# magenta/ddsp

Measured on NVIDIA H100. Metric: audio samples/sec (Harmonic+FilteredNoise decoder), higher is better.
Workload: dtype f32

## Files before the change

### ddsp_b200/csrc/noise_ring.cuh

```cuda
#pragma once
#include "noise_fused.cuh"

namespace ddsp {

namespace nr_ {
constexpr int NB = 65, FRAME = 64, S = 128, S0 = 128, Q = 32, SHIFT = 64;
constexpr int R = 16;
constexpr int UPT = FRAME / R;
constexpr int CONS_WARPS = 8, PROD_GROUPS = 3;
constexpr int GROUP_WARPS = 4, PROD_WARPS = GROUP_WARPS * PROD_GROUPS;
constexpr int NTG = CONS_WARPS / UPT;
static_assert((NTG & (NTG - 1)) == 0, "tile groups: a power of two");
constexpr int SLOTS = 7;
static_assert(SLOTS > NTG + 1, "the ring must leave slots to the producers");
constexpr int RING = 32 * SLOTS;
constexpr int THREADS = 32 * (CONS_WARPS + PROD_WARPS);
static_assert(THREADS <= 640, "noise_ring: the FIR needs 96 registers per thread");
constexpr int HPAD = 2, HS = 134, XS = 66, MS = 65;
constexpr int NQ = FRAME / 4;

constexpr int E_STEPS = 9, O_STEPS = 8;
constexpr int E_NT = 5, O_NT = 4;
constexpr int TAB_E = E_STEPS * E_NT * 32, TAB = TAB_E + O_STEPS * O_NT * 32;
__host__ __device__ constexpr int ir_kk(int s, int t) { return 16 * (s >> 2) + 4 * t + (s & 3); }

#ifdef DDSP_NR_TIMING
#define NR_TIMING_DECL unsigned tprev__ = (unsigned)clock()
__device__ unsigned g_nr_timing[kMaxSMs * 32 * 8];
#define NR_LAP(i)                                                                       \
  do {                                                                                  \
    const unsigned n__ = (unsigned)clock();                                             \
    if (lane == 0) atomicAdd(&g_nr_timing[(blockIdx.x * 32 + warp) * 8 + (i)], n__ - tprev__); \
    tprev__ = n__;                                                                      \
  } while (0)
#else
#define NR_TIMING_DECL
#define NR_LAP(i)
#endif

struct Smem {
  double ctab[TAB];
  float win[S];
  alignas(16) float raw[PROD_GROUPS][32 * NB + 8];
  alignas(16) float h[RING * HS];
  alignas(16) float x[RING * XS];
  alignas(8) unsigned long long full[SLOTS], empty[SLOTS], rawbar[PROD_GROUPS];
};

struct Params {
  const float* __restrict__ mags;
  const float* __restrict__ noise;
  float* audio;
  uint64_t seed, offset;
  int B, F, N, accumulate, raw, item_base;
  float bias;
};

struct Seg {
  int b, s0, len, nP, nC;
};

__device__ __forceinline__ bool next_seg(long long& g, long long g1, int F, Seg& sg) {
  if (g >= g1) return false;
  sg.b = (int)(g / F);
  sg.s0 = (int)(g - (long long)sg.b * F);
  sg.len = (int)min((long long)(F - sg.s0), g1 - g);
  sg.nP = (sg.len + 3 + 31) >> 5;
  sg.nC = (sg.len + 31) >> 5;
  g += sg.len;
  return true;
}

__device__ __forceinline__ void mbar_arrive_n(void* bar, int n) {
  asm volatile("mbarrier.arrive.shared::cta.b64 _, [%0], %1;" ::"r"(smem_u32(bar)),
               "r"(n)
               : "memory");
}

__device__ __forceinline__ float4 lds128v(const float* p) {
  float4 v;
  asm volatile("ld.shared.v4.f32 {%0, %1, %2, %3}, [%4];"
               : "=f"(v.x), "=f"(v.y), "=f"(v.z), "=f"(v.w)
               : "r"(smem_u32(p)));
  return v;
}
__device__ __forceinline__ float lds32v(const float* p) {
  float v;
  asm volatile("ld.shared.f32 %0, [%1];" : "=f"(v) : "r"(smem_u32(p)));
  return v;
}

__device__ __forceinline__ void dmma_16x8x4(double (&d)[4], double a0, double a1, double b) {
  asm("mma.sync.aligned.m16n8k4.row.col.f64.f64.f64.f64 {%0, %1, %2, %3}, {%4, %5}, {%6}, "
      "{%0, %1, %2, %3};"
      : "+d"(d[0]), "+d"(d[1]), "+d"(d[2]), "+d"(d[3])
      : "d"(a0), "d"(a1), "d"(b));
}

__device__ __forceinline__ void red_add_v4(float* addr, float a, float b, float c,
                                           float d) {
  asm volatile("red.global.add.v4.f32 [%0], {%1, %2, %3, %4};" ::"l"(addr), "f"(a),
               "f"(b), "f"(c), "f"(d)
               : "memory");
}

extern __shared__ __align__(16) unsigned char nr_smem[];
constexpr int X_OFF = (int)(offsetof(Smem, x) / 4), H_OFF = (int)(offsetof(Smem, h) / 4);
__device__ __forceinline__ float lds1(int off) {
  return reinterpret_cast<const float*>(nr_smem)[off];
}
__device__ __forceinline__ float2 lds2(int off) {
  return *reinterpret_cast<const float2*>(reinterpret_cast<const float*>(nr_smem) + off);
}

template <int D, int DLO, int DHI>
__device__ __forceinline__ void fir_diag(float (&y)[R], const float (&X)[R], float t) {
  if constexpr (D >= DLO && D <= DHI) {
#pragma unroll
    for (int k = (D < 0 ? -D : 0); k < (D > 0 ? R - D : R); ++k)
      y[k + D] = fmaf(X[k], t, y[k + D]);
  }
}
template <int J, int DLO, int DHI>
__device__ __forceinline__ void fir_pairs(float (&y)[R], const float (&X)[R], int ho) {
  if constexpr (2 * J + 1 >= DLO) {
    const float2 P = lds2(ho + 2 * J);
    fir_diag<2 * J + 1, DLO, DHI>(y, X, P.y);
    fir_diag<2 * J, DLO, DHI>(y, X, P.x);
    fir_pairs<J - 1, DLO, DHI>(y, X, ho);
  }
}
template <int DLO, int DHI>
__device__ __forceinline__ void fir_body(float (&y)[R], int xo, int ho) {
  float X[R];
#pragma unroll
  for (int k = 0; k < R; k += 2) {
    const float2 v = lds2(xo + k);
    X[k] = v.x;
    X[k + 1] = v.y;
  }
  fir_pairs<DHI / 2, DLO, DHI>(y, X, ho);
}

enum { OP_FULL = 0, OP_LOWER = 1, OP_UPPER = 2 };
constexpr int N_OPS = 2 * UPT + 1;

__device__ __forceinline__ void consume_unit(float (&y)[R], int u, const int (&xr)[4],
                                             const int (&hr)[4]) {
  const int N0 = R * u;
  const int xm1 = xr[0], hm1 = hr[0], x0 = xr[1], h0 = hr[1], xp1 = xr[2], hp1 = hr[2];
#pragma unroll 1
  for (int i = 0; i < N_OPS; ++i) {
    int kind = OP_FULL, xo, ho;
    if (i < UPT) {
      xo = x0 + R * i;
      ho = h0 + N0 + 62 - R * i;
    } else if (i < UPT + u) {
      const int j = i - UPT;
      xo = xm1 + R * j;
      ho = hm1 + N0 - 2 - R * j;
    } else if (i == UPT + u) {
      kind = OP_LOWER;
      xo = xm1 + N0;
      ho = hm1 - 2;
    } else if (i == UPT + u + 1) {
      kind = OP_UPPER;
      xo = xp1 + N0;
      ho = hp1 + 126;
    } else {
      const int j = i - UPT - 1;
      xo = xp1 + R * j;
      ho = hp1 + N0 + 126 - R * j;
    }
    switch (kind) {
      case OP_FULL: fir_body<-(R - 1), R - 1>(y, xo, ho); break;
      case OP_LOWER: fir_body<2, R - 1>(y, xo, ho); break;
      default: fir_body<-(R - 1), 1>(y, xo, ho); break;
    }
  }
  const int xe = u ? xp1 + N0 - 1 : xr[3] + 63, he = u ? hp1 + 127 : hr[3] + 127;
  y[0] = fmaf(lds1(xe), lds1(he), y[0]);
}
__global__ void __launch_bounds__(nr_::THREADS, 1)
noise_ring_kernel(Params p) {
  Smem& sm = *reinterpret_cast<Smem*>(nr_smem);
  const int tid = threadIdx.x, lane = tid & 31, warp = tid >> 5;

  for (int e = tid; e < TAB; e += THREADS) {
    const bool even = e < TAB_E;
    const int ee = even ? e : e - TAB_E, nts = even ? E_NT : O_NT;
    const int l = ee & 31, s = (ee >> 5) / nts, nt = (ee >> 5) - s * nts;
    const int kk = ir_kk(s, l & 3), k = even ? 2 * kk : 2 * kk + 1, n = 8 * nt + (l >> 2);
    double v = 0.0;
    if (k < NB && n <= Q) {
      const double ck = (k == 0 || k == NB - 1) ? 1.0 : 2.0;
      v = ck / S0 * cospi(2.0 * (double)((k * n) % S0) / S0);
    }
    sm.ctab[e] = v;
  }
  for (int j = tid; j < S; j += THREADS)
    sm.win[j] = 0.5f - 0.5f * cospif(2.0f * (float)j / (float)S0);
  for (int e = tid; e < RING * HS; e += THREADS) sm.h[e] = 0.f;
  for (int e = tid; e < RING * XS; e += THREADS) sm.x[e] = 0.f;
#ifdef DDSP_NR_TIMING
  for (int e = tid; e < 32 * 8; e += THREADS) g_nr_timing[blockIdx.x * 32 * 8 + e] = 0;
#endif
  if (tid == 0) {
    for (int i = 0; i < SLOTS; ++i) {
      mbar_init(&sm.full[i], GROUP_WARPS);
      mbar_init(&sm.empty[i], 2 * UPT);
    }
    for (int i = 0; i < PROD_GROUPS; ++i) mbar_init(&sm.rawbar[i], 1);
  }
  __syncthreads();

  const long long T = (long long)p.B * p.F;
  const long long g_lo = T * blockIdx.x / gridDim.x;
  const long long g_hi = T * (blockIdx.x + 1) / gridDim.x;

  if (warp < CONS_WARPS) {
    const int tg = warp / UPT, unit = warp % UPT;
    long long g = g_lo;
    Seg sg;
    int pbase = 0, ct = 0;
    bool dep_done = false;
    NR_TIMING_DECL;
    while (next_seg(g, g_hi, p.F, sg)) {
      for (int t = (tg - ct) & (NTG - 1); t < sg.nC; t += NTG) {
        NR_LAP(3);
        {
          const int P0 = pbase + t, P1 = pbase + min(t + 1, sg.nP - 1);
          mbar_wait(&sm.full[P0 % SLOTS], (P0 / SLOTS) & 1);
          mbar_wait(&sm.full[P1 % SLOTS], (P1 / SLOTS) & 1);
        }
        NR_LAP(0);
        const int q_rel = 32 * t + lane;
        const int rho = min(q_rel, sg.len - 1) + 2;
        const int rbase = pbase * 32;
        int xr[4], hr[4];
#pragma unroll
        for (int s = 0; s < 4; ++s) {
          const int row = (rbase + rho + 1 - s) % RING;
          xr[s] = X_OFF + row * XS;
          hr[s] = H_OFF + row * HS + HPAD;
        }
        float y[R];
#pragma unroll
        for (int c = 0; c < R; ++c) y[c] = 0.f;
        consume_unit(y, unit, xr, hr);
        __syncwarp();
        NR_LAP(1);
        if (lane == 0) {
#pragma unroll
          for (int d = 0; d < 2; ++d) {
            const int tau = t + d;
            if (tau < sg.nP) {
              const int readers = (tau >= 1 ? 1 : 0) + (tau < sg.nC ? 1 : 0);
              mbar_arrive_n(&sm.empty[(pbase + tau) % SLOTS], 2 / readers);
            }
          }
        }
        if (!dep_done) {
          asm volatile("griddepcontrol.wait;" ::: "memory");
          dep_done = true;
        }
        if (q_rel < sg.len) {
          constexpr int NOUT = R;
          const long long t0 = (long long)(sg.s0 + q_rel) * FRAME + NOUT * unit;
          float* o = p.audio + (size_t)sg.b * p.N + t0;
          if (t0 + NOUT <= p.N && (reinterpret_cast<uintptr_t>(o) & 15) == 0) {
#pragma unroll
            for (int w4 = 0; w4 < NOUT / 4; ++w4) {
              if (p.accumulate)
                red_add_v4(o + 4 * w4, y[4 * w4], y[4 * w4 + 1], y[4 * w4 + 2],
                           y[4 * w4 + 3]);
              else
                *reinterpret_cast<float4*>(o + 4 * w4) =
                    make_float4(y[4 * w4], y[4 * w4 + 1], y[4 * w4 + 2], y[4 * w4 + 3]);
            }
          } else {
#pragma unroll
            for (int w1 = 0; w1 < NOUT; ++w1) {
              if (t0 + w1 < p.N) {
                if (p.accumulate) o[w1] += y[w1]; else o[w1] = y[w1];
              }
            }
          }
        }
        NR_LAP(2);
      }
      ct += sg.nC;
      pbase += sg.nP;
    }
  } else {
    const int grp = (warp - CONS_WARPS) / GROUP_WARPS;
    const int iw = (warp - CONS_WARPS) % GROUP_WARPS;
    const int ptid = tid - (CONS_WARPS + GROUP_WARPS * grp) * 32;
    constexpr int PT = 32 * GROUP_WARPS;
    const int bar_id = 1 + grp;
    float* s_raw = sm.raw[grp];
    void* rawbar = &sm.rawbar[grp];
    const float* mags_end = p.mags + (size_t)p.B * p.F * NB;
    auto prefetch = [&](const Seg& s, int tau) -> int {
      const int jb = s.s0 - 2 + 32 * tau;
      const int r_lo = max(0, -jb), r_hi = min(32, p.F - jb);
      if (r_hi <= r_lo) {
        if (ptid == 0) mbar_arrive(rawbar);
        return 0;
      }
      const float* src = p.mags + ((size_t)s.b * p.F + jb + r_lo) * NB;
      const uintptr_t a = reinterpret_cast<uintptr_t>(src);
      const int off = (int)((a & 15) >> 2);
      const uint32_t bytes = (uint32_t)(((off + (r_hi - r_lo) * NB) * 4 + 15) & ~15);
      const uintptr_t a_al = a & ~(uintptr_t)15;
      if (a_al >= reinterpret_cast<uintptr_t>(p.mags) &&
          a_al + bytes <= reinterpret_cast<uintptr_t>(mags_end)) {
        if (ptid == 0) {
          mbar_expect_tx(rawbar, bytes);
          tma_bulk_g2s(s_raw, reinterpret_cast<const void*>(a_al), bytes, rawbar);
        }
        return off - r_lo * NB;
      }
      for (int e = ptid; e < (r_hi - r_lo) * NB; e += PT) cp_async4(s_raw + e, src + e);
      cp_async_wait_all();
      named_bar(bar_id, PT);
      if (ptid == 0) mbar_arrive(rawbar);
      return -r_lo * NB;
    };
    struct It {
      long long g;
      Seg sg;
      int tau, P;
      bool ok;
    };
    auto it_begin = [&]() {
      It it;
      it.g = g_lo; it.tau = 0; it.P = 0;
      it.ok = next_seg(it.g, g_hi, p.F, it.sg);
      return it;
    };
    auto it_next = [&](It& it) {
      ++it.P;
      if (++it.tau >= it.sg.nP) {
        it.tau = 0;
        it.ok = next_seg(it.g, g_hi, p.F, it.sg);
      }
    };
    It cur = it_begin();
    for (int i = 0; i < grp && cur.ok; ++i) it_next(cur);
    int roff = 0;
    if (cur.ok) roff = prefetch(cur.sg, cur.tau);
    int n_mine = 0;
    NR_TIMING_DECL;
    while (cur.ok) {
      NR_LAP(7);
      It nxt = cur;
      for (int i = 0; i < PROD_GROUPS && nxt.ok; ++i) it_next(nxt);
      const Seg& sg = cur.sg;
      const int P = cur.P, slot = P % SLOTS;
      const int jb = sg.s0 - 2 + 32 * cur.tau;
      mbar_wait(rawbar, n_mine & 1);
      NR_LAP(0);
      const bool row_ok = (jb + lane >= 0) && (jb + lane < p.F);
      if (p.raw && row_ok) {
        float* src = s_raw + roff + lane * NB + iw * 17;
        float v[17];
#pragma unroll
        for (int k = 0; k < 17; ++k) v[k] = (iw * 17 + k < NB) ? src[k] : 0.f;
#pragma unroll
        for (int k = 0; k < 17; ++k) v[k] = exp_sigmoid_f(v[k] + p.bias);
#pragma unroll
        for (int k = 0; k < 17; ++k)
          if (iw * 17 + k < NB) src[k] = v[k];
      }
      named_bar(bar_id, PT);
      ++n_mine;
      NR_LAP(1);
      const float* nzb = p.noise ? p.noise + (size_t)sg.b * p.N : nullptr;
      const uint32_t item = (uint32_t)(sg.b + p.item_base);
      const long long p_lo = (long long)jb * FRAME;
      const bool interior = (jb >= 0) && (jb + 32 <= p.F) &&
                            (p_lo + 32ll * FRAME <= p.N) && !nzb;
      constexpr int PER = 32 * NQ / 4;
      {
        const int g = lane >> 2, t = lane & 3;
        const int ntb = 2 * (iw & 1);
        const bool mid = iw & 1;
        const int f0 = 16 * (iw >> 1) + g, f1 = f0 + 8;
        const bool ok0 = (jb + f0 >= 0) && (jb + f0 < p.F);
        const bool ok1 = (jb + f1 >= 0) && (jb + f1 < p.F);
        const float* m0 = ok0 ? s_raw + roff + f0 * NB : s_raw;
        const float* m1 = ok1 ? s_raw + roff + f1 * NB : s_raw;
        const double* tb = sm.ctab + lane;
        double aE[3][4], aO[2][4];
#pragma unroll
        for (int c = 0; c < 4; ++c) {
          aE[0][c] = aE[1][c] = aE[2][c] = 0.0;
          aO[0][c] = aO[1][c] = 0.0;
        }
#pragma unroll
        for (int s = 0; s < E_STEPS; ++s) {
          const int k = 2 * ir_kk(s, t);
          const bool kin = s < E_STEPS - 1 || k < NB;
          const double e0 = kin ? (double)m0[k] : 0.0, e1 = kin ? (double)m1[k] : 0.0;
          dmma_16x8x4(aE[0], e0, e1, tb[(s * E_NT + ntb) * 32]);
          dmma_16x8x4(aE[1], e0, e1, tb[(s * E_NT + ntb + 1) * 32]);
          if (mid) dmma_16x8x4(aE[2], e0, e1, tb[(s * E_NT + 4) * 32]);
          if (s < O_STEPS) {
            const double o0 = m0[k + 1], o1 = m1[k + 1];
            dmma_16x8x4(aO[0], o0, o1, tb[TAB_E + (s * O_NT + ntb) * 32]);
            dmma_16x8x4(aO[1], o0, o1, tb[TAB_E + (s * O_NT + ntb + 1) * 32]);
          }
        }
        NR_LAP(3);
        named_bar(bar_id, PT);
        if (nxt.ok) roff = prefetch(nxt.sg, nxt.tau);
        NR_LAP(4);
        if (P >= SLOTS) mbar_wait(&sm.empty[slot], ((P / SLOTS) - 1) & 1);
        NR_LAP(2);
        float* hs = sm.h + slot * 32 * HS + HPAD;
#pragma unroll
        for (int j = 0; j < 2; ++j) {
          const int n = 8 * (ntb + j) + 2 * t;
          const float2 wp = *reinterpret_cast<const float2*>(sm.win + SHIFT + n);
          const float2 wm = *reinterpret_cast<const float2*>(sm.win + n);
#pragma unroll
          for (int r = 0; r < 2; ++r) {
            const bool ok = r ? ok1 : ok0;
            float* hr = hs + (r ? f1 : f0) * HS;
            const double E0 = aE[j][2 * r], E1 = aE[j][2 * r + 1];
            const double O0 = aO[j][2 * r], O1 = aO[j][2 * r + 1];
            const float p0 = ok ? wp.x * (float)(E0 + O0) : 0.f;
            const float p1 = ok ? wp.y * (float)(E1 + O1) : 0.f;
            const float q0 = ok ? wm.x * (float)(E0 - O0) : 0.f;
            const float q1 = ok ? wm.y * (float)(E1 - O1) : 0.f;
            *reinterpret_cast<float2*>(hr + SHIFT + n) = make_float2(p0, p1);
            hr[SHIFT - n] = p0;
            hr[SHIFT - n - 1] = p1;
            *reinterpret_cast<float2*>(hr + n) = make_float2(q0, q1);
            if (n != 0) hr[S - n] = q0;
            hr[S - n - 1] = q1;
          }
        }
        if (mid && t == 0) {
#pragma unroll
          for (int r = 0; r < 2; ++r) {
            const float v = (r ? ok1 : ok0) ? sm.win[Q] * (float)aE[2][2 * r] : 0.f;
            float* hr = hs + (r ? f1 : f0) * HS;
            hr[Q] = v;
            hr[S - Q] = v;
          }
        }
      }
      NR_LAP(5);
      {
        float* xs = sm.x + slot * 32 * XS;
        if (interior) {
          const uint32_t qbase = (uint32_t)(p_lo >> 2);
#pragma unroll
          for (int it = 0; it < PER / 32; ++it) {
            const int e = iw * PER + it * 32 + lane;
            const int r = e >> 4, qd = e & 15;
            const float4 v = noise4(qbase + (uint32_t)e, item, p.seed, p.offset);
            float2* d = reinterpret_cast<float2*>(xs + r * XS + 4 * qd);
            d[0] = make_float2(v.x, v.y);
            d[1] = make_float2(v.z, v.w);
          }
        } else {
          for (int it = 0; it < PER / 32; ++it) {
            const int e = iw * PER + it * 32 + lane;
            const int r = e >> 4, qd = e & 15;
            const int j = jb + r;
            const long long pp = (long long)j * FRAME + 4 * qd;
            float v[4] = {0.f, 0.f, 0.f, 0.f};
            if (j >= 0 && j < p.F && pp < p.N) {
              if (nzb) {
#pragma unroll
                for (int u = 0; u < 4; ++u) if (pp + u < p.N) v[u] = nzb[pp + u];
              } else {
                const float4 r4 = noise4((uint32_t)(pp >> 2), item, p.seed, p.offset);
                v[0] = r4.x;
                if (pp + 1 < p.N) v[1] = r4.y;
                if (pp + 2 < p.N) v[2] = r4.z;
                if (pp + 3 < p.N) v[3] = r4.w;
              }
            }
            float2* d = reinterpret_cast<float2*>(xs + r * XS + 4 * qd);
            d[0] = make_float2(v[0], v[1]);
            d[1] = make_float2(v[2], v[3]);
          }
        }
      }
      __syncwarp();
      if (lane == 0) mbar_arrive(&sm.full[slot]);
      NR_LAP(6);
      cur = nxt;
    }
  }
}

}

inline bool noise_ring_supported(int F, int nb, int N, int window_size) {
  if (nb != nr_::NB) return false;
  if (N % F != 0 || N / F != nr_::FRAME) return false;
  IrGeom g = make_ir_geom(nb, window_size);
  return !g.padded && g.S == nr_::S;
}

inline int launch_noise_ring(const float* mags, const float* noise, uint64_t seed,
                             uint64_t offset, float* audio, int B, int F, int N,
                             int accumulate, cudaStream_t st, int raw, float bias,
                             int item_base, int overlap_previous = 0) {
  nr_::Params p;
  p.mags = mags; p.noise = noise; p.audio = audio; p.seed = seed; p.offset = offset;
  p.B = B; p.F = F; p.N = N; p.accumulate = accumulate; p.raw = raw; p.bias = bias;
  p.item_base = item_base;
  const long long T = (long long)B * F;
  const size_t smem = sizeof(nr_::Smem);
  static_assert(sizeof(nr_::Smem) <= 227 * 1024, "noise_ring shared memory");
  int rc = set_smem(nr_::noise_ring_kernel, smem, "filtered_noise_forward");
  if (rc) return rc;
  const int grid = (int)std::max<long long>(
      1, std::min<long long>((long long)num_sms(), (T + 31) / 32));
  cudaLaunchConfig_t cfg = {};
  cfg.gridDim = dim3(grid);
  cfg.blockDim = dim3(nr_::THREADS);
  cfg.dynamicSmemBytes = smem;
  cfg.stream = st;
  cudaLaunchAttribute attr[1];
  attr[0].id = cudaLaunchAttributeProgrammaticStreamSerialization;
  attr[0].val.programmaticStreamSerializationAllowed = overlap_previous ? 1 : 0;
  cfg.attrs = attr;
  cfg.numAttrs = 1;
  cudaError_t e = cudaLaunchKernelEx(&cfg, nr_::noise_ring_kernel, p);
  if (e != cudaSuccess) {
    set_error("filtered_noise_forward(ring): launch failed: %s", cudaGetErrorString(e));
    return DDSP_B200_E_CUDA;
  }
  DDSP_CHECK_LAUNCH("filtered_noise_forward(ring)");
  return 0;
}

inline int launch_noise_best(const float* mags, const float* noise, uint64_t seed,
                             uint64_t offset, float* audio, int B, int F, int nb,
                             int N, int window_size, int accumulate,
                             cudaStream_t st, int raw = 0, float bias = 0.f,
                             int item_base = 0, int overlap_previous = 0) {
  if (noise_ring_supported(F, nb, N, window_size))
    return launch_noise_ring(mags, noise, seed, offset, audio, B, F, N, accumulate,
                             st, raw, bias, item_base, overlap_previous);
  return launch_noise_fused(mags, noise, seed, offset, audio, B, F, nb, N,
                            window_size, accumulate, st, raw, bias, item_base);
}

}
```

Before: 48.58 billion.

## Vectorize FIR shared-memory loads and reuse filter taps across consecutive ops

```diff
diff --git a/ddsp_b200/csrc/noise_ring.cuh b/ddsp_b200/csrc/noise_ring.cuh
--- a/ddsp_b200/csrc/noise_ring.cuh
+++ b/ddsp_b200/csrc/noise_ring.cuh
@@ -16,7 +16,7 @@
 constexpr int RING = 32 * SLOTS;
 constexpr int THREADS = 32 * (CONS_WARPS + PROD_WARPS);
 static_assert(THREADS <= 640, "noise_ring: the FIR needs 96 registers per thread");
-constexpr int HPAD = 2, HS = 134, XS = 66, MS = 65;
+constexpr int HPAD = 2, HS = 132, XS = 68, MS = 65;
 constexpr int NQ = FRAME / 4;
 
 constexpr int E_STEPS = 9, O_STEPS = 8;
@@ -49,6 +49,7 @@
 
 struct Params {
   const float* __restrict__ mags;
+  const float* mags_end;
   const float* __restrict__ noise;
   float* audio;
   uint64_t seed, offset;
@@ -112,6 +113,9 @@
 __device__ __forceinline__ float2 lds2(int off) {
   return *reinterpret_cast<const float2*>(reinterpret_cast<const float*>(nr_smem) + off);
 }
+__device__ __forceinline__ float4 lds4(int off) {
+  return *reinterpret_cast<const float4*>(reinterpret_cast<const float*>(nr_smem) + off);
+}
 
 template <int D, int DLO, int DHI>
 __device__ __forceinline__ void fir_diag(float (&y)[R], const float (&X)[R], float t) {
@@ -122,24 +126,44 @@
   }
 }
 template <int J, int DLO, int DHI>
-__device__ __forceinline__ void fir_pairs(float (&y)[R], const float (&X)[R], int ho) {
-  if constexpr (2 * J + 1 >= DLO) {
-    const float2 P = lds2(ho + 2 * J);
-    fir_diag<2 * J + 1, DLO, DHI>(y, X, P.y);
-    fir_diag<2 * J, DLO, DHI>(y, X, P.x);
-    fir_pairs<J - 1, DLO, DHI>(y, X, ho);
+__device__ __forceinline__ void fir_pair(float (&y)[R], const float (&X)[R], float2 P) {
+  fir_diag<2 * J + 1, DLO, DHI>(y, X, P.y);
+  fir_diag<2 * J, DLO, DHI>(y, X, P.x);
+}
+template <int J, int DLO, int DHI>
+__device__ __forceinline__ void fir_hi(float (&y)[R], const float (&X)[R],
+                                       const float2 (&T)[R / 2]) {
+  if constexpr (J >= 0 && 2 * J + 1 >= DLO) {
+    fir_pair<J, DLO, DHI>(y, X, T[J]);
+    fir_hi<J - 1, DLO, DHI>(y, X, T);
+  }
+}
+template <int J, int DLO, int DHI>
+__device__ __forceinline__ void fir_lo(float (&y)[R], const float (&X)[R],
+                                       float2 (&T)[R / 2], int ho) {
+  if constexpr (J >= -R / 2 && 2 * J + 1 >= DLO) {
+    if constexpr (J & 1) {
+      const float4 q = lds4(ho + 2 * (J - 1));
+      T[J - 1 + R / 2] = make_float2(q.x, q.y);
+      T[J + R / 2] = make_float2(q.z, q.w);
+    }
+    fir_pair<J, DLO, DHI>(y, X, T[J + R / 2]);
+    fir_lo<J - 1, DLO, DHI>(y, X, T, ho);
   }
 }
 template <int DLO, int DHI>
-__device__ __forceinline__ void fir_body(float (&y)[R], int xo, int ho) {
+__device__ __forceinline__ void fir_body(float (&y)[R], float2 (&T)[R / 2], int xo, int ho) {
   float X[R];
 #pragma unroll
-  for (int k = 0; k < R; k += 2) {
-    const float2 v = lds2(xo + k);
+  for (int k = 0; k < R; k += 4) {
+    const float4 v = lds4(xo + k);
     X[k] = v.x;
     X[k + 1] = v.y;
-  }
-  fir_pairs<DHI / 2, DLO, DHI>(y, X, ho);
+    X[k + 2] = v.z;
+    X[k + 3] = v.w;
+  }
+  fir_hi<R / 2 - 1, DLO, DHI>(y, X, T);
+  fir_lo<-1, DLO, DHI>(y, X, T, ho);
 }
 
 enum { OP_FULL = 0, OP_LOWER = 1, OP_UPPER = 2 };
@@ -149,20 +173,25 @@
                                              const int (&hr)[4]) {
   const int N0 = R * u;
   const int xm1 = xr[0], hm1 = hr[0], x0 = xr[1], h0 = hr[1], xp1 = xr[2], hp1 = hr[2];
+  float2 T[R / 2];
 #pragma unroll 1
   for (int i = 0; i < N_OPS; ++i) {
     int kind = OP_FULL, xo, ho;
+    bool start = false;
     if (i < UPT) {
       xo = x0 + R * i;
       ho = h0 + N0 + 62 - R * i;
+      start = i == 0;
     } else if (i < UPT + u) {
       const int j = i - UPT;
       xo = xm1 + R * j;
       ho = hm1 + N0 - 2 - R * j;
+      start = j == 0;
     } else if (i == UPT + u) {
       kind = OP_LOWER;
       xo = xm1 + N0;
       ho = hm1 - 2;
+      start = u == 0;
     } else if (i == UPT + u + 1) {
       kind = OP_UPPER;
       xo = xp1 + N0;
@@ -172,10 +201,21 @@
       xo = xp1 + R * j;
       ho = hp1 + N0 + 126 - R * j;
     }
+    if (start) {
+#pragma unroll
+      for (int j = 0; j < R / 2; j += 2) {
+        const float4 q = lds4(ho + 2 * j);
+        T[j] = make_float2(q.x, q.y);
+        T[j + 1] = make_float2(q.z, q.w);
+      }
+    }
     switch (kind) {
-      case OP_FULL: fir_body<-(R - 1), R - 1>(y, xo, ho); break;
-      case OP_LOWER: fir_body<2, R - 1>(y, xo, ho); break;
-      default: fir_body<-(R - 1), 1>(y, xo, ho); break;
+      case OP_FULL: fir_body<-(R - 1), R - 1>(y, T, xo, ho); break;
+      case OP_LOWER: fir_body<2, R - 1>(y, T, xo, ho); break;
+      default:
+        T[0] = lds2(ho);
+        fir_body<-(R - 1), 1>(y, T, xo, ho);
+        break;
     }
   }
   const int xe = u ? xp1 + N0 - 1 : xr[3] + 63, he = u ? hp1 + 127 : hr[3] + 127;
@@ -300,7 +340,6 @@
     const int bar_id = 1 + grp;
     float* s_raw = sm.raw[grp];
     void* rawbar = &sm.rawbar[grp];
-    const float* mags_end = p.mags + (size_t)p.B * p.F * NB;
     auto prefetch = [&](const Seg& s, int tau) -> int {
       const int jb = s.s0 - 2 + 32 * tau;
       const int r_lo = max(0, -jb), r_hi = min(32, p.F - jb);
@@ -314,7 +353,7 @@
       const uint32_t bytes = (uint32_t)(((off + (r_hi - r_lo) * NB) * 4 + 15) & ~15);
       const uintptr_t a_al = a & ~(uintptr_t)15;
       if (a_al >= reinterpret_cast<uintptr_t>(p.mags) &&
-          a_al + bytes <= reinterpret_cast<uintptr_t>(mags_end)) {
+          a_al + bytes <= reinterpret_cast<uintptr_t>(p.mags_end)) {
         if (ptid == 0) {
           mbar_expect_tx(rawbar, bytes);
           tma_bulk_g2s(s_raw, reinterpret_cast<const void*>(a_al), bytes, rawbar);
@@ -461,10 +500,8 @@
           for (int it = 0; it < PER / 32; ++it) {
             const int e = iw * PER + it * 32 + lane;
             const int r = e >> 4, qd = e & 15;
-            const float4 v = noise4(qbase + (uint32_t)e, item, p.seed, p.offset);
-            float2* d = reinterpret_cast<float2*>(xs + r * XS + 4 * qd);
-            d[0] = make_float2(v.x, v.y);
-            d[1] = make_float2(v.z, v.w);
+            *reinterpret_cast<float4*>(xs + r * XS + 4 * qd) =
+                noise4(qbase + (uint32_t)e, item, p.seed, p.offset);
           }
         } else {
           for (int it = 0; it < PER / 32; ++it) {
@@ -485,9 +522,8 @@
                 if (pp + 3 < p.N) v[3] = r4.w;
               }
             }
-            float2* d = reinterpret_cast<float2*>(xs + r * XS + 4 * qd);
-            d[0] = make_float2(v[0], v[1]);
-            d[1] = make_float2(v[2], v[3]);
+            *reinterpret_cast<float4*>(xs + r * XS + 4 * qd) =
+                make_float4(v[0], v[1], v[2], v[3]);
           }
         }
       }
@@ -514,6 +550,7 @@
                              int item_base, int overlap_previous = 0) {
   nr_::Params p;
   p.mags = mags; p.noise = noise; p.audio = audio; p.seed = seed; p.offset = offset;
+  p.mags_end = mags + (size_t)B * F * nr_::NB;
   p.B = B; p.F = F; p.N = N; p.accumulate = accumulate; p.raw = raw; p.bias = bias;
   p.item_base = item_base;
   const long long T = (long long)B * F;
```

Result: faster. 49.35 billion, median of 6 (+1.6%).
